# jacklishufan/InstructAny2Pix

Hardware: AMD Instinct MI355X
Metric: denoise-steps/sec (512x512, 50-step DDIM, batch 8) (higher is better)
Workload: dtype f16; 1 GPU; BASELINE configs[2]: 512x512, latent [8,4,64,64], 50-step DDIM, ctx 81 (77 text + 4 IP tokens), SDXL-base UNet + IP-Adapter; global_batch=8, parallelism=dp1, context_kv=projected in every step (reference schedule, as rounds 1-4), ranks=1, dist_backend=none (single process), weight_broadcast_route=none

## Files before the change

include/ia2p_debug.h:

```cpp
#ifndef IA2P_DEBUG_H
#define IA2P_DEBUG_H

#include "ia2p.h"

#ifdef __cplusplus
extern "C" {
#endif

void ia2p_debug_set_gemm_splitk(int splitk);
void ia2p_debug_invalidate_splitk_counters(void);
int ia2p_debug_fill_splitk_counters(void* stream, int value);
void ia2p_debug_set_splitk_inkernel(long long bytes);
void ia2p_debug_set_gn_plan(int mode);
void ia2p_debug_set_gemm_tile(int variant);
void ia2p_debug_set_xattn_min_tiles(int tiles);
void ia2p_debug_set_attn_fold(int mode);
int ia2p_debug_gemm_tile_info(int variant, int* out);
void ia2p_debug_gemm_plan(int M, int N, int K, int conv, int geglu, int* variant, int* splitk);

ia2p_status ia2p_profile_enable(ia2p_ctx* ctx, int on);
int ia2p_profile_classes(void);
ia2p_status ia2p_profile_read_prefetch(ia2p_ctx* ctx, int k, double* bytes);
ia2p_status ia2p_profile_read(ia2p_ctx* ctx, int k, char* name, int name_len, int64_t* launches, double* ms, double* flops, double* bytes);
ia2p_status ia2p_profile_read_region(ia2p_ctx* ctx, int region, int64_t* launches, double* ms, double* flops, double* bytes);
int ia2p_profile_roles(void);
ia2p_status ia2p_profile_read_role(ia2p_ctx* ctx, int role, char* name, int name_len, int64_t* launches, double* ms, double* flops, double* bytes);
ia2p_status ia2p_profile_read_role_class(ia2p_ctx* ctx, int role, int k, int64_t* launches, double* ms);

#ifdef __cplusplus
}
#endif
#endif
```

instructany2pix_amd/_ffi.py:

```python
from __future__ import annotations

import contextlib
import ctypes as C
import functools
import os

_HERE = os.path.dirname(os.path.abspath(__file__))
LIB_PATH = os.path.join(_HERE, "libia2p_hip.so")

IA2P_OK = 0
_STATUS_NAMES = {1: "INVALID", 2: "SHAPE", 3: "KEY", 4: "STATE", 5: "NOMEM", 6: "HIP", 7: "ARCH"}
MAX_BLOCKS = 4


class UNetConfigC(C.Structure):
    _fields_ = [
        ("in_channels", C.c_int), ("out_channels", C.c_int), ("n_blocks", C.c_int),
        ("block_out_channels", C.c_int * MAX_BLOCKS), ("transformer_layers_per_block", C.c_int * MAX_BLOCKS),
        ("num_heads", C.c_int * MAX_BLOCKS), ("layers_per_block", C.c_int), ("cross_attention_dim", C.c_int),
        ("norm_num_groups", C.c_int), ("norm_eps", C.c_float), ("addition_time_embed_dim", C.c_int),
        ("projection_class_embeddings_input_dim", C.c_int), ("time_embed_dim", C.c_int), ("time_proj_dim", C.c_int),
        ("mid_transformer_layers", C.c_int), ("num_time_ids", C.c_int),
    ]

# ... 77 lines not shown
    "ia2p_layernorm": (_I, [_P, _P, _P, _P, _P, _I, _I, _F]),
    "ia2p_gemm": (_I, [_P, _P, _P, _P, _P, _P, _I, _I, _I, _I]),
    "ia2p_gemm_splitk": (_I, [_P, _P, _P, _P, _P, _P, _I, _I, _I, _I, _P]),
    "ia2p_ffn": (_I, [_P, _P, _P, _P, _P, _P, _P, _P, _P, _I, _I, _I, _P]),
    "ia2p_fold_layernorm": (_I, [_P, _P, _P, _P, _P, _P, _P, _P, _I, _I]),
    "ia2p_gemm_ex": (_I, [_P, _P, _P, _P, _P, _P, _I, _I, _I, _I, _P, _P, _P, _I, _P]),
    "ia2p_debug_set_gemm_splitk": (None, [_I]),
    "ia2p_conv3x3": (_I, [_P, _P, _P, _P, _P, _P, _P, _I, _I, _I, _I, _I, _I, _I]),
    "ia2p_conv3x3_splitk": (_I, [_P, _P, _P, _P, _P, _P, _P, _I, _I, _I, _I, _I, _I, _P]),
    "ia2p_pack_conv3x3": (_I, [_P, _P, _P, _I, _I]),
    "ia2p_pack_conv_out": (_I, [_P, _P, _P, _I, _I]),
    "ia2p_conv3x3_cat": (_I, [_P, _P, _P, _P, _P, _P, _I, _I, _I, _I, _I, _I]),
    "ia2p_pack_geglu": (_I, [_P, _P, _P, _I, _I]),
    "ia2p_conv_in": (_I, [_P, _P, _P, _P, _P, _P, _I, _I, _I, _I, _I]),
    "ia2p_conv_out": (_I, [_P, _P, _P, _P, _P, _I, _I, _I, _I, _I]),
    "ia2p_attention": (_I, [_P, _P, _I, _P, _I, _I, _I, _I, _I, _P, _P, _I, _I, _F, _P, _P, _I, _I, _F]),
    "ia2p_qkv_self_attention": (_I, [_P, _P, _P, _P, _P, _P, _I, _I, _I, _I]),
    "ia2p_qkv_self_attention_ctx": (_I, [_P, _P, _P, _P, _P, _P, _I, _I, _I, _I, _P, _I, _I, _I, _P, _P, _P, _P, _I, _I, _P]),
    "ia2p_qproj_attention": (_I, [_P, _P, _P, _P, _P, _P, _I, _I, _I, _I, _I, _I, _P, _P, _I, _I, _F, _P, _P, _I, _I, _F]),
    "ia2p_linear_small": (_I, [_P, _P, _P, _P, _P, _I, _I, _I, _I, _I]),
    "ia2p_ip_attn_map": (_I, [_P, _P, _I, _P, _I, _P, _I, _I, _I, _I]),
    "ia2p_debug_set_gemm_tile": (None, [_I]),
    "ia2p_debug_gemm_tile_info": (_I, [_I, _P]),
    "ia2p_debug_set_xattn_min_tiles": (None, [_I]),
    "ia2p_debug_set_attn_fold": (None, [_I]),
    "ia2p_debug_set_splitk_inkernel": (None, [C.c_longlong]),
    "ia2p_debug_invalidate_splitk_counters": (None, []),
    "ia2p_debug_fill_splitk_counters": (_I, [_P, _I]),
    "ia2p_debug_gemm_plan": (None, [_I, _I, _I, _I, _I, _P, _P]),
    "ia2p_clip_create": (_I, [C.POINTER(CLIPConfigC), C.POINTER(_P)]),
    "ia2p_clip_destroy": (None, [_P]),
    "ia2p_clip_last_error": (C.c_char_p, [_P]),
    "ia2p_clip_arena_bytes": (_SZ, [_P]),
    "ia2p_clip_bind_arena": (_I, [_P, _P, _SZ]),
    "ia2p_clip_load_tensor": (_I, [_P, C.c_char_p, _P, C.POINTER(C.c_int64), _I, _P]),
    "ia2p_clip_finalize_weights": (_I, [_P]),
    "ia2p_clip_workspace_bytes": (_SZ, [_P, _I, _I]),
    "ia2p_clip_encode": (_I, [_P, _P, _P, _I, _I, _P, _P, _P, _P, _SZ]),
    "ia2p_clip_encode_embeds": (_I, [_P, _P, _P, _I, _I, _P, _P, _P, _SZ]),
    "ia2p_vit_create": (_I, [C.POINTER(ViTConfigC), C.POINTER(_P)]),
    "ia2p_vit_destroy": (None, [_P]),
    "ia2p_vit_last_error": (C.c_char_p, [_P]),
    "ia2p_vit_arena_bytes": (_SZ, [_P]),
    "ia2p_vit_tokens": (_I, [_P]),
    "ia2p_vit_bind_arena": (_I, [_P, _P, _SZ]),
    "ia2p_vit_load_tensor": (_I, [_P, C.c_char_p, _P, C.POINTER(C.c_int64), _I, _P]),
# ... 319 lines not shown
```

instructany2pix_amd/csrc/conv_halo_kernel.h:

```cpp
#pragma once
#include "gemm_epilogue.h"

template <int BN> struct HaloWaves { static constexpr int WGM = BN == 80 ? 8 : 4, WGN = BN == 80 ? 1 : 2; };

template <int BN, int GN> struct HaloSmem {
  using BS = BStage<BN, 64, 8, 1>;
  static constexpr int H_BASE = 3 * BS::BNL * 128, H_BYTES = 48 * 1024;
  static constexpr int GN_GSTAT = H_BASE + 2 * H_BYTES, GN_TBL = GN_GSTAT + 512, GN_ZERO = GN_TBL + 512, LOOP = GN ? GN_ZERO + 512 : H_BASE + 2 * H_BYTES;
  static constexpr int EPI = EpiCfg<256, BN, 3, HaloWaves<BN>::WGM, 64, HaloWaves<BN>::WGN, 1>::SMEM;
  static constexpr int SMEM = LOOP > EPI ? LOOP : EPI;
  static_assert(SMEM <= 160 * 1024, "halo-staged tile exceeds the CU's LDS");
};

struct GnOp { int step, e; };
constexpr int GN_NOPS = 32;
constexpr GnOp GN_OPS[GN_NOPS] = {{0, 0}, {0, 1}, {0, 2}, {1, 0}, {0, 3}, {1, 1}, {2, 0}, {0, 4}, {1, 2}, {2, 1}, {3, 0}, {0, 5}, {1, 3}, {2, 2}, {3, 1}, {0, 6},
                                  {1, 4}, {2, 3}, {3, 2}, {0, 7}, {1, 5}, {2, 4}, {3, 3}, {1, 6}, {2, 5}, {3, 4}, {1, 7}, {2, 6}, {3, 5}, {2, 7}, {3, 6}, {3, 7}};

template <int BN, int GN>
__device__ __forceinline__ void conv_halo_tile_body(const half_t* hA, const half_t* hW, int hM, int hN, int hK, int hlda, int hldw, int hsplitk, int hgroup_w, int hmfast, int gHo, int gWo, int gHs, int gWs,
                                                    int gUp, int gCin, int gCin2, const GemmArgs& p) {
  constexpr int BM = 256, BK = 64, NSTAGE = 3, PP = 1, WGM = HaloWaves<BN>::WGM, WGN = HaloWaves<BN>::WGN;
  constexpr int NWAVE = WGM * WGN;
  static_assert(NWAVE == 8, "ping-pong schedule: 8 waves (two groups of 4 by tile rows)");
// ... 413 lines not shown
  tile_epilogue<BM, BN, NSTAGE, WGM, BK, PP, WGN, 0, 1>(acc, tc, p, nullptr, kvr);
}

template <int BN, int GN = 0>
__global__ __launch_bounds__(512, 2) void conv_halo_f16_kernel(const half_t* hA, const half_t* hW, int hM, int hN, int hK, int hlda, int hldw, int hsk_gw, int hHoWo, int hHsWs, int hUpCin,
                                                                 int hCin2, const GemmArgs p) {
  conv_halo_tile_body<BN, GN>(hA, hW, hM, hN, hK, hlda, hldw, IA2P_SKGW_LO8(hsk_gw), IA2P_SKGW_GW(hsk_gw), IA2P_SKGW_FLAGS(hsk_gw) & 1, hHoWo & 0xffff, (int)((unsigned)hHoWo >> 16), hHsWs & 0xffff,
                              (int)((unsigned)hHsWs >> 16), hUpCin & 3, (int)((unsigned)hUpCin >> 2), hCin2, p);
}

template <int BN, int GN>
static hipError_t launch_halo_gn(const GemmArgs& a, hipStream_t s) {
  constexpr int smem = HaloSmem<BN, GN>::SMEM;
  static bool attr_set[64] = {false};
  int dev = 0;
  (void)hipGetDevice(&dev);
  if (dev < 0 || dev >= 64 || !attr_set[dev]) {
    hipError_t e = hipFuncSetAttribute((const void*)conv_halo_f16_kernel<BN, GN>, hipFuncAttributeMaxDynamicSharedMemorySize, smem);
    if (e != hipSuccess) return e;
    if (dev >= 0 && dev < 64) attr_set[dev] = true;
  }
  const int tiles = (a.M / 256) * ((a.N + BN - 1) / BN);
  GemmArgs b = a;
  ia2p_gemm_prepare(b, smem, 256, BN, true);
  if (b.gn_out && !b.vec8) return hipErrorInvalidValue;
  if (b.sk_counters && tiles > ia2p_sk_counter_capacity()) return hipErrorInvalidValue;
  if ((long)tiles * (a.splitk > 1 ? a.splitk : 1) >= (1L << 21)) return hipErrorInvalidValue;
  int sk_gw, howo, hsws;
  if (!ia2p_pack_skgw(b.splitk, b.group_w, b.m_fastest, false, &sk_gw) || !ia2p_pack_rowmap(b.Ho, b.Wo, &howo) || !ia2p_pack_rowmap(b.Hs, b.Ws, &hsws) || b.up < 0 || b.up > 3 || b.Cin < 0 || b.Cin >= (1 << 29))
    return hipErrorInvalidValue;
  hipLaunchKernelGGL((conv_halo_f16_kernel<BN, GN>), dim3(tiles * (a.splitk > 1 ? a.splitk : 1)), dim3(512), smem, s,
                     b.A, b.W, b.M, b.N, b.K, b.lda, b.ldw, sk_gw, howo, hsws, (int)((unsigned)b.up | ((unsigned)b.Cin << 2)), b.Cin2, b);
  return hipGetLastError();
}
template <int BN>
static hipError_t launch_halo(const GemmArgs& a, hipStream_t s) {
  if (!ia2p_conv_halo_ok(a) || !ia2p_conv_gn_ok(a)) return hipErrorInvalidValue;
  return a.gn.st0 ? launch_halo_gn<BN, 1>(a, s) : launch_halo_gn<BN, 0>(a, s);
}
```

instructany2pix_amd/csrc/gemm.hip:

```cpp
#include "gemm_kernel.h"
#include "conv_halo_kernel.h"
#include "gemm_geglu_kernel.h"

#include <algorithm>
#include <atomic>
#include <cmath>
#include <cstdio>
#include <cstdlib>
#include <cstring>
#include <map>
#include <mutex>
#include <string>
#include <tuple>
#include <vector>


static std::mutex g_plan_mu;
static unsigned long long g_plan_gen = 0;
static void plan_gen_bump() { std::lock_guard<std::mutex> lk(g_plan_mu); ++g_plan_gen; }
static int g_force_variant = -1;
extern "C" void ia2p_debug_set_gemm_tile(int v) { if (v != g_force_variant) plan_gen_bump(); g_force_variant = v; }
extern "C" int ia2p_debug_gemm_tile_info(int v, int* out) {
  if (v < 0 || v >= IA2P_GEMM_NVARIANT || !out) return -1;
  out[0] = IA2P_GEMM_TILES[v].bm; out[1] = IA2P_GEMM_TILES[v].bn; out[2] = IA2P_GEMM_TILES[v].stages; out[3] = IA2P_GEMM_TILES[v].halo ? 3 : IA2P_GEMM_TILES[v].pp;
// ... 62 lines not shown
#pragma unroll
        for (int r = 0; r < 4; ++r) { const float f = (float)o[r]; st1 += f; st2 += f * f; }
      }
    }
    if (hstats_out) {
#pragma unroll
      for (int o = 32; o > 0; o >>= 1) { st1 += __shfl_xor(st1, o); st2 += __shfl_xor(st2, o); }
      if (lane == 0) ((float2*)hstats_out)[m] = make_float2(st1, st2);
    }
  }
}

static long long g_sk_limit = -1;
extern "C" void ia2p_debug_set_splitk_inkernel(long long bytes) { g_sk_limit = bytes; }
bool ia2p_splitk_inkernel(int M, int N, int splitk) {
  static const size_t env_limit = getenv("IA2P_SPLITK_INKERNEL") ? (size_t)atoll(getenv("IA2P_SPLITK_INKERNEL")) : ((size_t)1 << 46);
  const size_t limit = g_sk_limit >= 0 ? (size_t)g_sk_limit : env_limit;
  return splitk > 1 && (size_t)splitk * M * N * sizeof(float) <= limit;
}
static int g_force_gn = -1;
extern "C" void ia2p_debug_set_gn_plan(int v) { if (v != g_force_gn) plan_gen_bump(); g_force_gn = v; }
static int g_force_splitk = -1;
extern "C" void ia2p_debug_set_gemm_splitk(int s) { if (s != g_force_splitk) plan_gen_bump(); g_force_splitk = s; }

static constexpr int POOL_INTS = 1 << 18, POOL_SK = POOL_INTS - 4096;
int ia2p_sk_counter_capacity() { return POOL_SK; }
static std::atomic<unsigned> g_sk_epoch{1};
void ia2p_sk_counters_invalidate() { g_sk_epoch.fetch_add(1, std::memory_order_relaxed); }
extern "C" void ia2p_debug_invalidate_splitk_counters(void) { ia2p_sk_counters_invalidate(); }
static int* pool_buffer(hipStream_t s) {
  struct Entry { int* p; unsigned epoch; };
  static std::mutex mu;
  static std::map<std::pair<int, hipStream_t>, Entry> pool;
  int dev = 0;
  if (hipGetDevice(&dev) != hipSuccess) return nullptr;
  const unsigned epoch = g_sk_epoch.load(std::memory_order_relaxed);
  const size_t bytes = (size_t)POOL_INTS * sizeof(int);
  std::lock_guard<std::mutex> lk(mu);
  auto it = pool.find({dev, s});
  if (it != pool.end()) {
    if (it->second.p && it->second.epoch != epoch) {
      if (hipMemsetAsync(it->second.p, 0, bytes, s) != hipSuccess) { (void)hipGetLastError(); return nullptr; }
      it->second.epoch = epoch;
    }
    return it->second.p;
  }
// ... 306 lines not shown
```

instructany2pix_amd/csrc/gemm_geglu_kernel.h:

```cpp
#pragma once
#include "gemm_tile.h"

struct Geglu320 {
  static constexpr int BM = 256, BN = 320, BK = 64, NWAVE = 8, WGN = 2, WM = 64, WN = 160, MR = 4, NR = 10;
  static constexpr int ROWB = 128, RPP = 8, A_PW = 4, B_PW = 5;
  static constexpr int STAGE = (BM + BN) * ROWB, RING = 2 * STAGE;
  static constexpr int HN = BN / 2, P16 = HN * 2 + 16, T16_BYTES = BM * P16;
  static constexpr int CONST_BYTES = 2 * BN * 4, LUT_BYTES = (IA2P_PHI_LUT_N * 8 + 15) & ~15, LNROW_BYTES = 2 * BM * 4;
  static_assert(T16_BYTES <= RING, "the output tile lives inside the ring");
  static constexpr int SMEM = RING + LNROW_BYTES + CONST_BYTES + LUT_BYTES;
  static_assert(SMEM <= 160 * 1024 && A_PW * NWAVE * RPP == BM && B_PW * NWAVE * RPP == BN, "LDS budget / staging split");
};

__global__ __launch_bounds__(512, 2) void gemm_geglu_f16_kernel(const half_t* hA, const half_t* hW, const float* h_ln_stats, const float* h_ln_cs, int hM, int hN, int hK, int hlda, int hldw,
                                                               int h_slots_gw, const GemmArgs p) {
  const int h_ln_slots = IA2P_SKGW_LO8(h_slots_gw), hgroup_w = IA2P_SKGW_GW(h_slots_gw), h_m_fastest = IA2P_SKGW_FLAGS(h_slots_gw) & 1;
  using G = Geglu320;
  constexpr int BM = G::BM, BN = G::BN, MR = G::MR, NR = G::NR, ROWB = G::ROWB, RPP = G::RPP, A_PW = G::A_PW, B_PW = G::B_PW, STAGE = G::STAGE, NT = G::NWAVE * 64;
  extern __shared__ __attribute__((aligned(1024))) char smem[];
  const int tid = threadIdx.x;
  const int lane = tid & 63;
  const int wave = __builtin_amdgcn_readfirstlane(tid >> 6);
  const __amdgpu_buffer_rsrc_t rs_a = __builtin_amdgcn_make_buffer_rsrc((void*)hA, 0, 0x7ffffe00, 0x00020000);
  const __amdgpu_buffer_rsrc_t rs_w = __builtin_amdgcn_make_buffer_rsrc((void*)hW, 0, 0x7ffffe00, 0x00020000);
// ... 289 lines not shown
    if (tid == 0 && p.partial) ((unsigned long long*)p.partial)[8 * blockIdx.x + 6] = __builtin_amdgcn_s_memrealtime();
    asm volatile("s_waitcnt vmcnt(0)" ::: "memory");
    __syncthreads();
    if (tid == 0 && p.partial) ((unsigned long long*)p.partial)[8 * blockIdx.x + 5] = __builtin_amdgcn_s_memrealtime();
  )
}

static inline bool ia2p_geglu320_ok(const GemmArgs& a) {
  return a.geglu && a.splitk <= 1 && !a.act && !a.residual && !a.rowvec && !a.stats_out && !a.gn_out && !a.gn.st0 && a.K >= 64 && a.K % 64 == 0 && a.M > 0 && a.M % Geglu320::BM == 0 &&
         a.N > 0 && a.N % Geglu320::BN == 0 && !a.rpb && (a.bias || a.ln_stats);
}
static hipError_t launch_geglu320(const GemmArgs& a, hipStream_t s) {
  using G = Geglu320;
  if (!ia2p_geglu320_ok(a)) return hipErrorInvalidValue;
  static bool attr_set[64] = {false};
  int dev = 0;
  (void)hipGetDevice(&dev);
  if (dev < 0 || dev >= 64 || !attr_set[dev]) {
    hipError_t e = hipFuncSetAttribute((const void*)gemm_geglu_f16_kernel, hipFuncAttributeMaxDynamicSharedMemorySize, G::SMEM);
    if (e != hipSuccess) return e;
    if (dev >= 0 && dev < 64) attr_set[dev] = true;
  }
  GemmArgs b = a;
  ia2p_gemm_prepare(b, G::SMEM, G::BM, G::BN, false);
  if (!b.vec8) return hipErrorInvalidValue;
  if (!b.phi_lut) return hipErrorOutOfMemory;
  const size_t a_rows = a.rpb ? ((size_t)a.M / a.rpb + 1) * (size_t)std::max(a.bstride, 0) + a.roff + a.rpb : (size_t)a.M;
  if (!ia2p_fits_buffer(a_rows, a.lda) || !ia2p_fits_buffer(a.N, a.ldw)) return hipErrorInvalidValue;
  if ((a.ln_stats && ((((uintptr_t)a.ln_cs) | ((uintptr_t)a.ln_bias)) & 15)) || (!a.ln_stats && (((uintptr_t)a.bias) & 7))) return hipErrorInvalidValue;
  b.splitk = 0; b.sk_counters = nullptr;
#ifndef IA2P_CLOCK_STAMP
  b.partial = nullptr;
#endif
  const int tiles = ((a.M + G::BM - 1) / G::BM) * ((a.N + G::BN - 1) / G::BN);
  if (tiles >= (1 << 21)) return hipErrorInvalidValue;
  int slots_gw;
  if (!ia2p_pack_skgw(b.ln_stats ? b.ln_slots : 0, b.group_w, b.m_fastest, b.ln_stats != nullptr, &slots_gw)) return hipErrorInvalidValue;
  hipLaunchKernelGGL(gemm_geglu_f16_kernel, dim3(tiles), dim3(512), G::SMEM, s, b.A, b.W, b.ln_stats, b.ln_cs, b.M, b.N, b.K, b.lda, b.ldw, slots_gw, b);
  return hipGetLastError();
}
```

instructany2pix_amd/csrc/gemm_kernel.h:

```cpp
#pragma once
#include "gemm_epilogue.h"

template <int BM, int BN, int NSTAGE, bool CONV, int WGM = 2, int BK = 64, int PP = 0, int WGN = 2, int XA = 0, bool SUB = false>
__device__ __forceinline__ void gemm_tile_body(const half_t* hA, const half_t* hW, const half_t* hzero, int hM, int hN, int hK, int hlda, int hldw, int hrpb, int hbstride,
                                               int hroff, int hsplitk, int hgroup_w, int hflags, const GemmArgs& p, const AttnArgs* xa, const float* pre_ln_stats = nullptr, int pre_ln_slots = 0, int bid0 = 0) {
  static_assert(PP != 1 || (WGM * WGN == 8 && (WGM == 4 || WGM == 8) && NSTAGE == 3), "ping-pong schedule: 8 waves (two groups of 4 by tile rows), 3-stage ring");
  static_assert(PP != 3 || (WGM == 4 && NSTAGE == 2 && !CONV), "two-slot ping-pong schedule: 8 waves, 2 k-tile slots");
  static_assert(PP != 2 || (WGM == 2 && WGN == 4 && NSTAGE == 2 && BK == 64 && BM == 256 && (BN == 256 || BN == 128) && XA == 0), "8-phase schedule: 256-row tiles, 2 x 4 waves, two k-tile buffers");
  constexpr int NWAVE = WGM * WGN;
  constexpr int WM = BM / WGM, WN = BN / WGN;
  constexpr int MR = WM / 16, NR = WN / 16;
  constexpr int ROWB = 2 * BK, CPR = ROWB / 16, RPP = 1024 / ROWB;
  using BS = BStage<BN, BK, NWAVE, PP>;
  constexpr int A_PW = BM / RPP / NWAVE, B_PW = BS::HI;
  constexpr bool B_UNEVEN = BS::UNEVEN;
  constexpr int BNL = BS::BNL;
  static_assert(BM % (RPP * NWAVE) == 0 && BN % 16 == 0 && WN % 16 == 0 && WM % 16 == 0, "tile / wave layout");
  constexpr int STAGE = (BM + BNL) * ROWB;
  constexpr int KSUB = BK / 32;
  extern __shared__ __attribute__((aligned(1024))) char smem[];

  int tid_ = threadIdx.x;
  if constexpr (SUB) asm volatile("" : "+v"(tid_));
  const int tid = tid_;
// ... 570 lines not shown
  )
  tile_epilogue<BM, BN, NSTAGE, WGM, BK, PP, WGN, XA, 0>(acc, tc, p, xa, kvr);
}

template <int BM, int BN, int NSTAGE, bool CONV, int WGM = 2, int BK = 64, int PP = 0, int WGN = 2>
__global__ __launch_bounds__(WGM * WGN * 64, 2) void gemm_f16_kernel(const half_t* hA, const half_t* hW, const half_t* hzero, int hM, int hN, int hK, int hlda, int hldw, int hrowmap,
                                                                         int hbstride, int hsk_gw, const GemmArgs p) {
  gemm_tile_body<BM, BN, NSTAGE, CONV, WGM, BK, PP, WGN, 0>(hA, hW, hzero, hM, hN, hK, hlda, hldw, hrowmap & 0xffff, hbstride, (int)((unsigned)hrowmap >> 16), IA2P_SKGW_LO8(hsk_gw),
                                                            IA2P_SKGW_GW(hsk_gw), IA2P_SKGW_FLAGS(hsk_gw), p, nullptr);
}
template <int BM, int BN, int NSTAGE, bool CONV, int WGM = 2, int BK = 64, int PP = 0, int WGN = 2>
static hipError_t launch_cfg(const GemmArgs& a, hipStream_t s) {
  constexpr int smem = EpiCfg<BM, BN, NSTAGE, WGM, BK, WGN, PP>::SMEM;
  static bool attr_set[64] = {false};
  int dev = 0;
  (void)hipGetDevice(&dev);
  if (dev < 0 || dev >= 64 || !attr_set[dev]) {
    hipError_t e = hipFuncSetAttribute((const void*)gemm_f16_kernel<BM, BN, NSTAGE, CONV, WGM, BK, PP, WGN>, hipFuncAttributeMaxDynamicSharedMemorySize, smem);
    if (e != hipSuccess) return e;
    if (dev >= 0 && dev < 64) attr_set[dev] = true;
  }
  const int tiles = ((a.M + BM - 1) / BM) * ((a.N + BN - 1) / BN);
  GemmArgs b = a;
  ia2p_gemm_prepare(b, smem, BM, BN, CONV);
  if (a.geglu && !b.vec8) return hipErrorInvalidValue;
  if (a.gn.st0) return hipErrorInvalidValue;
  if (a.gn_out && (!b.vec8 || a.geglu)) return hipErrorInvalidValue;
  if (a.geglu && !b.phi_lut) return hipErrorOutOfMemory;
  if (!CONV && IA2P_LIN_BUF) {
    const size_t a_rows = a.rpb ? ((size_t)a.M / a.rpb + 1) * (size_t)std::max(a.bstride, 0) + a.roff + a.rpb : (size_t)a.M;
    if (!ia2p_fits_buffer(a_rows, a.lda) || !ia2p_fits_buffer(a.N, a.ldw)) return hipErrorInvalidValue;
  }
  if (b.sk_counters && tiles > ia2p_sk_counter_capacity()) return hipErrorInvalidValue;
  const int extra = (!PP && a.pf && a.pf_bytes >= 4096) ? a.pf_blocks : 0;
  if ((long)tiles * (a.splitk > 1 ? a.splitk : 1) + extra >= (1L << 21)) return hipErrorInvalidValue;
  int rowmap, sk_gw;
  if (!ia2p_pack_rowmap(b.rpb, b.roff, &rowmap) || !ia2p_pack_skgw(b.splitk, b.group_w, b.m_fastest, b.ln_stats != nullptr, &sk_gw)) return hipErrorInvalidValue;
  hipLaunchKernelGGL((gemm_f16_kernel<BM, BN, NSTAGE, CONV, WGM, BK, PP, WGN>), dim3(tiles * (a.splitk > 1 ? a.splitk : 1) + extra), dim3(WGM * WGN * 64), smem, s,
                     b.A, b.W, b.zero, b.M, b.N, b.K, b.lda, b.ldw, rowmap, b.bstride, sk_gw, b);
  return hipGetLastError();
}
```

instructany2pix_amd/csrc/gemm_tile.h:

```cpp
#pragma once
#include "common.h"
#include "attention_core.h"

#include <algorithm>
#include <cmath>
#include <cstdint>
#include <cstdlib>
#include <type_traits>

bool ia2p_splitk_inkernel(int M, int N, int splitk);
int ia2p_gemm_variant_ran(const GemmArgs& a, bool conv, int v);
int ia2p_sk_counter_capacity();
int* ia2p_sk_counters(hipStream_t s, int tiles);
void ia2p_sk_counters_invalidate();
const float* ia2p_phi_lut();

#ifndef IA2P_LIN_BUF
#define IA2P_LIN_BUF 1
#endif
#define BLDS16(rsrc, ldsptr, voff, soff) \
  __builtin_amdgcn_raw_ptr_buffer_load_lds(rsrc, (__attribute__((address_space(3))) void*)(ldsptr), 16, voff, soff, 0, 0)
#define GLDS16(gptr, ldsptr)                                                                         \
  __builtin_amdgcn_global_load_lds((const __attribute__((address_space(1))) void*)(gptr),            \
                                   (__attribute__((address_space(3))) void*)(ldsptr), 16, 0, 0)

// ... 47 lines not shown

#ifdef IA2P_CLOCK_STAMP
#define IA2P_STAMP(...) __VA_ARGS__
#ifndef IA2P_STAMP_AT
#define IA2P_STAMP_AT 0
#endif
__device__ __forceinline__ unsigned long long* stamp_base(const GemmArgs& p, int nsplit) {
  return p.stamp ? p.stamp : (nsplit == 1 ? (unsigned long long*)p.partial : nullptr);
}
__device__ __forceinline__ void stamp_put(const GemmArgs& p, int nsplit, int slot) {
  unsigned long long* b = stamp_base(p, nsplit);
  if (threadIdx.x == 0 && b) b[8 * blockIdx.x + slot] = __builtin_amdgcn_s_memrealtime();
}
#else
#define IA2P_STAMP(...)
#endif

__device__ __forceinline__ int udiv_small(int a, int b) {
  int q = (int)((float)a * __builtin_amdgcn_rcpf((float)b));
  const int r = a - q * b;
  q += (r >= b ? 1 : 0) - (r < 0 ? 1 : 0);
  return q;
}
__device__ __forceinline__ void tile_order(int bid, int tiles_m, int tiles_n, int group_w, int m_fastest, int& tm, int& tn) {
  {
    const int nwg = tiles_m * tiles_n;
    const int q = nwg >> 3, r = nwg & 7, x = bid & 7, i = bid >> 3;
    bid = (x < r ? x * (q + 1) : r * (q + 1) + (x - r) * q) + i;
  }
  if (group_w > 0) {
    const int per = tiles_m * group_w;
    const int panel = udiv_small(bid, per), r = bid - panel * per;
    const int w = min(group_w, tiles_n - panel * group_w);
    tm = udiv_small(r, w); tn = panel * group_w + (r - tm * w);
  } else if (m_fastest) { tn = udiv_small(bid, tiles_m); tm = bid - tn * tiles_m; }
  else                  { tm = udiv_small(bid, tiles_n); tn = bid - tm * tiles_n; }
}

struct TileCtx {
  int hM, hN, hK;
  int tm, tn, bm0, bn0, tiles_m, tiles_n;
  int split, nsplit;
  int h_m0;
  float ln_s1, ln_s2;
#ifdef IA2P_CLOCK_STAMP
  unsigned long long stamp_c0, stamp_r0, stamp_entry;
#endif
};

static inline int ia2p_tile_group_w(int tiles, int tiles_n, int smem, double a_over_w) {
  static const int group_mode = getenv("IA2P_TILE_GROUP") ? atoi(getenv("IA2P_TILE_GROUP")) : 2;
  if (!group_mode) return 0;
  const int smem_per_cu = 160 * 1024 / smem;
  const double resident = std::min<double>(tiles / 8.0, 32.0 * std::max(1, std::min(smem_per_cu, 2)));
  static const double gscale = ia2p_exp_env("IA2P_TILE_GROUP_SCALE") ? atof(ia2p_exp_env("IA2P_TILE_GROUP_SCALE")) : 1.0;
  const int w = (int)(gscale * std::sqrt(resident * a_over_w) + 0.5);
  return std::max(1, std::min(w, tiles_n));
}
static inline int ia2p_tile_group_w(int tiles, int tiles_n, int smem, int BM, int BN) { return ia2p_tile_group_w(tiles, tiles_n, smem, (double)BM / BN); }

static inline bool ia2p_pack_rowmap(int rpb, int roff, int* out) {
  if (rpb < 0 || rpb > 0xffff || roff < 0 || roff > 0xffff) return false;
  *out = (int)((unsigned)rpb | ((unsigned)roff << 16));
  return true;
}
static inline bool ia2p_pack_skgw(int lo8, int group_w, int m_fastest, bool has_ln, int* out) {
  if (lo8 < 0 || lo8 > 0xff || group_w < 0 || group_w > 0x3fffff) return false;
  *out = (int)((unsigned)lo8 | (m_fastest ? 0x100u : 0u) | (has_ln ? 0x200u : 0u) | ((unsigned)group_w << 10));
  return true;
}
#define IA2P_SKGW_LO8(w) ((w) & 0xff)
#define IA2P_SKGW_FLAGS(w) (((w) >> 8) & 3)
#define IA2P_SKGW_GW(w) ((int)((unsigned)(w) >> 10))

static inline void ia2p_gemm_prepare(GemmArgs& b, int smem, int BM, int BN, bool conv = false) {
  auto al16 = [](const void* q) { return (((uintptr_t)q) & 15) == 0; };
  b.vec8 = (b.ldc % 8 == 0 && al16(b.C) && (!b.bias || al16(b.bias)) && (!b.residual || (b.ldr % 8 == 0 && al16(b.residual))) &&
            (!b.rowvec || (b.rowvec_ld % 8 == 0 && al16(b.rowvec)))) ? 1 : 0;
  b.c_wt = ((ia2p_wt_mask() & 1) && (size_t)b.M * b.ldc * 2 < (size_t)0x7ffffff0) ? 1 : 0;
  b.phi_lut = b.geglu ? ia2p_phi_lut() : nullptr;
  const int tiles_n = (b.N + BN - 1) / BN;
  double a_over_w = (double)BM / BN;
  static const int group_mode = getenv("IA2P_TILE_GROUP") ? atoi(getenv("IA2P_TILE_GROUP")) : 2;
  if (conv && group_mode >= 2 && b.K > 0)
    a_over_w = BM * (1.5 * b.Cin + (b.A2 ? b.Cin2 : 0) + (b.A3 ? b.Cin3 : 0)) / ((double)BN * b.K);
  b.group_w = ia2p_tile_group_w(((b.M + BM - 1) / BM) * tiles_n, tiles_n, smem, a_over_w);
}
```

instructany2pix_amd/csrc/qxattn.hip:

```cpp
#include "gemm_kernel.h"
#include "launch_args.h"

#include <cstring>

#ifndef IA2P_QX_STAGES
#define IA2P_QX_STAGES 2
#endif
template <int MODE>
__global__ __launch_bounds__(256, 2) void qproj_xattn_kernel(const half_t* hA, const half_t* hW, const half_t* hzero, const float* h_ln_stats, int hM, int hN, int hK, int hlda, int hldw,
                                                             int h_slots_gw, const GemmArgs p, const AttnArgs xa) {
  gemm_tile_body<128, 64, IA2P_QX_STAGES, false, 2, 64, 0, 2, MODE + 1>(hA, hW, hzero, hM, hN, hK, hlda, hldw, 0, 0, 0, 0, IA2P_SKGW_GW(h_slots_gw), IA2P_SKGW_FLAGS(h_slots_gw), p, &xa, h_ln_stats,
                                                                        IA2P_SKGW_LO8(h_slots_gw));
}

bool ia2p_qproj_xattn_ok(const GemmArgs& a, const AttnArgs& x) {
  return x.Nq > 0 && x.Nq % 128 == 0 && a.M == x.B * x.Nq && a.N == x.heads * 64 && a.K >= 64 && a.K % 64 == 0 && a.splitk <= 1 && !a.rpb && !a.geglu && !a.residual && !a.rowvec &&
         !a.stats_out && !a.act && x.nseg >= 1 && x.nseg <= 2 && x.seg[0].nkeys > 0 && (x.nseg == 1 || x.seg[1].nkeys > 0) &&
         (!a.bias || ((((uintptr_t)a.bias) & 15) == 0 && a.N % 8 == 0)) && x.ldo % 8 == 0 && ((((uintptr_t)x.O) & 15) == 0) &&
         ia2p_fits_buffer(a.rpb ? ((size_t)a.M / a.rpb + 1) * (size_t)(a.bstride > 0 ? a.bstride : 0) + a.roff + a.rpb : (size_t)a.M, a.lda) && ia2p_fits_buffer(a.N, a.ldw) &&
         attn_kv_resident(x);
}

hipError_t ia2p_launch_qproj_xattn(const GemmArgs& a, const AttnArgs& x, hipStream_t s) {
  if (!ia2p_qproj_xattn_ok(a, x)) return hipErrorInvalidValue;
  constexpr int BM = 128, BN = 64, SMEM = EpiCfg<128, 64, IA2P_QX_STAGES, 2, 64, 2>::SMEM > 65536 ? EpiCfg<128, 64, IA2P_QX_STAGES, 2, 64, 2>::SMEM : 65536;
  static_assert(EpiCfg<BM, BN, IA2P_QX_STAGES, 2, 64, 2>::SMEM <= SMEM, "LDS budget");
  static bool attr_set[64] = {false};
  int dev = 0;
  (void)hipGetDevice(&dev);
  if (dev < 0 || dev >= 64 || !attr_set[dev]) {
    hipError_t e = hipFuncSetAttribute((const void*)qproj_xattn_kernel<0>, hipFuncAttributeMaxDynamicSharedMemorySize, SMEM);
    if (e == hipSuccess) e = hipFuncSetAttribute((const void*)qproj_xattn_kernel<1>, hipFuncAttributeMaxDynamicSharedMemorySize, SMEM);
    if (e == hipSuccess) e = hipFuncSetAttribute((const void*)qproj_xattn_kernel<2>, hipFuncAttributeMaxDynamicSharedMemorySize, SMEM);
    if (e != hipSuccess) return e;
    if (dev >= 0 && dev < 64) attr_set[dev] = true;
  }
  const int tiles_n = a.N / BN, tiles = (a.M / BM) * tiles_n;
  GemmArgs b = a;
  b.vec8 = 1; b.splitk = 0; b.sk_counters = nullptr;
#ifndef IA2P_CLOCK_STAMP
  b.partial = nullptr;
#endif
  b.group_w = ia2p_tile_group_w(tiles, tiles_n, SMEM, BM, BN);
  AttnArgs y = x;
  y.xcd_map = (((ia2p_wt_mask() & 8) && (size_t)x.B * x.Nq * x.ldo * 2 < (size_t)0x7ffffff0) ? 2 : 0) | (ia2p_attn_fold_enabled() ? 0 : 4);
  const int extra = (a.pf && a.pf_bytes >= 4096) ? a.pf_blocks : 0;
  int slots_gw;
  if (tiles + extra >= (1 << 21) || !ia2p_pack_skgw(b.ln_stats ? b.ln_slots : 0, b.group_w, b.m_fastest, b.ln_stats != nullptr, &slots_gw)) return hipErrorInvalidValue;
  const int mode = y.nseg == 1 ? 0 : (y.seg[1].nkeys <= 64 && y.seg[0].weight != 0.f) ? 1 : 2;
#define IA2P_QX_LAUNCH(MODE)                                                                                                                   \
  hipLaunchKernelGGL(qproj_xattn_kernel<MODE>, dim3(tiles + extra), dim3(256), SMEM, s, b.A, b.W, b.zero, b.ln_stats, b.M, b.N, b.K, b.lda, b.ldw, slots_gw, b, y)
  if (mode == 0) IA2P_QX_LAUNCH(0);
  else if (mode == 1) IA2P_QX_LAUNCH(1);
  else IA2P_QX_LAUNCH(2);
#undef IA2P_QX_LAUNCH
  return hipGetLastError();
}


__global__ __launch_bounds__(512, 2) void qkv_sattn_kernel(const half_t* hA, const half_t* hW, const half_t* hzero, const float* h_ln_stats, int hM, int hN, int hK, int hlda, int hldw,
                                                           int h_slots_gw, const GemmArgs p, const AttnArgs xa, const CtxKvArgs ck) {
#ifndef IA2P_SATTN_PP
#define IA2P_SATTN_PP 3
#endif
  gemm_tile_body<256, 192, 2, false, 4, 64, IA2P_SATTN_PP, 2, 4>(hA, hW, hzero, hM, hN, hK, hlda, hldw, 0, 0, 0, 0, IA2P_SKGW_GW(h_slots_gw), IA2P_SKGW_FLAGS(h_slots_gw), p, &xa, h_ln_stats, IA2P_SKGW_LO8(h_slots_gw));
}
// ... 20 lines not shown
  const int tn = (k.N + CK_BN - 1) / CK_BN;
  return ((k.B * k.Lt + CK_BM - 1) / CK_BM) * tn + (k.Li > 0 ? ((k.B * k.Li + CK_BM - 1) / CK_BM) * tn : 0);
}
bool ia2p_qkv_sattn_ctx_ok(const AttnArgs& x, const CtxKvSlice& k) {
  if (k.B < 1 || k.B != x.B || k.Lt < 1 || k.Li < 0 || k.L != k.Lt + k.Li || k.N < 8 || k.N % 8 || k.K < 64 || k.K % 64 || k.lda < k.K || k.ldc < k.N) return false;
  if (k.Lt > 0xffff || k.Li > 0xffff || (long)k.B * k.L >= (1L << 21)) return false;
  if (!ia2p_fits_buffer((size_t)k.B * k.L + k.L, k.lda) || !ia2p_fits_buffer(k.N, k.K)) return false;
  return (long)x.B * x.heads + ia2p_qkv_sattn_ctx_tiles(k) <= ia2p_cu_count();
}

hipError_t ia2p_launch_qkv_sattn(const GemmArgs& a, const AttnArgs& x, hipStream_t s, const CtxKvSlice* ctx) {
  if (!ia2p_qkv_sattn_ok(a, x)) return hipErrorInvalidValue;
  constexpr int SMEM = EpiCfg<256, 192, 2, 4, 64, 2, 0>::SMEM;
  static_assert(SMEM >= 96 * 1024 + (2 * 256 + 2 * 192) * 4, "K / V / Q images + row and column constants");
  constexpr int CK_SMEM = EpiCfg<CK_BM, CK_BN, 3, 4, 64, 2, 1>::SMEM;
  static_assert(CK_SMEM <= SMEM, "a context K/V tile runs in the fused tile's LDS request");
  CtxKvArgs ck;
  memset(&ck, 0, sizeof ck);
  if (ctx) {
    if (!ia2p_qkv_sattn_ctx_ok(x, *ctx) || !ctx->ctx || !ctx->Wt || !ctx->Ct || (ctx->Li > 0 && (!ctx->Wi || !ctx->Ci))) return hipErrorInvalidValue;
    const int tn = (ctx->N + CK_BN - 1) / CK_BN;
    auto fill = [&](GemmArgs& g, const half_t* W, half_t* C, int rows, int roff) {
      g = gemm_desc(a.zero, ctx->ctx, ctx->lda, W, ctx->K, nullptr, nullptr, 0, C, ctx->ldc, ctx->B * rows, ctx->N, ctx->K, 0, rows, ctx->L, roff);
      ia2p_gemm_prepare(g, CK_SMEM, CK_BM, CK_BN);
    };
    fill(ck.g[0], ctx->Wt, ctx->Ct, ctx->Lt, 0);
    ck.nt[0] = ((ck.g[0].M + CK_BM - 1) / CK_BM) * tn;
    if (ctx->Li > 0) {
      fill(ck.g[1], ctx->Wi, ctx->Ci, ctx->Li, ctx->Lt);
      ck.nt[1] = ((ck.g[1].M + CK_BM - 1) / CK_BM) * tn;
    }
  }
  static bool attr_set[64] = {false};
  int dev = 0;
  (void)hipGetDevice(&dev);
  if (dev < 0 || dev >= 64 || !attr_set[dev]) {
    hipError_t e = hipFuncSetAttribute((const void*)qkv_sattn_kernel, hipFuncAttributeMaxDynamicSharedMemorySize, SMEM);
    if (e != hipSuccess) return e;
    if (dev >= 0 && dev < 64) attr_set[dev] = true;
  }
  const int tiles_n = x.heads, tiles = x.B * tiles_n;
  GemmArgs b = a;
  b.vec8 = 1; b.splitk = 0; b.sk_counters = nullptr;
#ifndef IA2P_CLOCK_STAMP
  b.partial = nullptr;
#endif
  b.m_fastest = 0;
  b.group_w = ia2p_tile_group_w(tiles, tiles_n, SMEM, 256, 192);
  AttnArgs y = x;
  y.seg[0].nkeys = 256; y.seg[0].weight = 1.f; y.nseg = 1;
  y.xcd_map = ((ia2p_wt_mask() & 8) && (size_t)x.B * x.Nq * x.ldo * 2 < (size_t)0x7ffffff0) ? 2 : 0;
  const int extra = (a.pf && a.pf_bytes >= 4096) ? a.pf_blocks : 0;
  const int nct = ck.nt[0] + ck.nt[1];
  int slots_gw;
  if (tiles + nct + extra >= (1 << 21) || !ia2p_pack_skgw(b.ln_stats ? b.ln_slots : 0, b.group_w, b.m_fastest, b.ln_stats != nullptr, &slots_gw)) return hipErrorInvalidValue;
  hipLaunchKernelGGL(qkv_sattn_kernel, dim3(tiles + nct + extra), dim3(512), SMEM, s, b.A, b.W, b.zero, b.ln_stats, b.M, b.N, b.K, b.lda, b.ldw, slots_gw, b, y, ck);
  return hipGetLastError();
}
```

Measured before the change: 55.05 steps/s.

## Choose GEMM tile-group width by exact simulation of resident panel traffic

Adds a host-side search that simulates which tile rows and columns are resident per XCD wave for each candidate group width, then picks the width that minimizes estimated A/W panel fetch bytes. This is now the default (mode 3) and replaces the closed-form sqrt rule. Residency is derived from LDS use and thread count per launch, and results are cached per shape. It also factors the tile map into a shared host/device header and adds debug probes. The risk is host-side cost on first use, and mispredicted grouping that could raise L2 traffic for some shapes.

```diff
diff --git a/include/ia2p_debug.h b/include/ia2p_debug.h
--- a/include/ia2p_debug.h
+++ b/include/ia2p_debug.h
@@ -15,6 +15,10 @@
 void ia2p_debug_set_gemm_tile(int variant);
 void ia2p_debug_set_xattn_min_tiles(int tiles);
 void ia2p_debug_set_attn_fold(int mode);
+void ia2p_debug_set_tile_group(int mode);
+void ia2p_debug_set_tile_group_w(int w);
+int ia2p_debug_tile_order(void* stream, int tiles_m, int tiles_n, int group_w, int m_fastest, int* out);
+int ia2p_debug_tile_order_host(int tiles_m, int tiles_n, int group_w, int m_fastest, int* out);
 int ia2p_debug_gemm_tile_info(int variant, int* out);
 void ia2p_debug_gemm_plan(int M, int N, int K, int conv, int geglu, int* variant, int* splitk);
 
diff --git a/instructany2pix_amd/_ffi.py b/instructany2pix_amd/_ffi.py
--- a/instructany2pix_amd/_ffi.py
+++ b/instructany2pix_amd/_ffi.py
@@ -123,6 +123,10 @@
     "ia2p_ip_attn_map": (_I, [_P, _P, _I, _P, _I, _P, _I, _I, _I, _I]),
     "ia2p_debug_set_gemm_tile": (None, [_I]),
     "ia2p_debug_gemm_tile_info": (_I, [_I, _P]),
+    "ia2p_debug_set_tile_group": (None, [_I]),
+    "ia2p_debug_set_tile_group_w": (None, [_I]),
+    "ia2p_debug_tile_order": (_I, [_P, _I, _I, _I, _I, _P]),
+    "ia2p_debug_tile_order_host": (_I, [_I, _I, _I, _I, _P]),
     "ia2p_debug_set_xattn_min_tiles": (None, [_I]),
     "ia2p_debug_set_attn_fold": (None, [_I]),
     "ia2p_debug_set_splitk_inkernel": (None, [C.c_longlong]),
diff --git a/instructany2pix_amd/csrc/conv_halo_kernel.h b/instructany2pix_amd/csrc/conv_halo_kernel.h
--- a/instructany2pix_amd/csrc/conv_halo_kernel.h
+++ b/instructany2pix_amd/csrc/conv_halo_kernel.h
@@ -459,7 +459,7 @@
   }
   const int tiles = (a.M / 256) * ((a.N + BN - 1) / BN);
   GemmArgs b = a;
-  ia2p_gemm_prepare(b, smem, 256, BN, true);
+  ia2p_gemm_prepare(b, smem, 512, 256, BN, true);
   if (b.gn_out && !b.vec8) return hipErrorInvalidValue;
   if (b.sk_counters && tiles > ia2p_sk_counter_capacity()) return hipErrorInvalidValue;
   if ((long)tiles * (a.splitk > 1 ? a.splitk : 1) >= (1L << 21)) return hipErrorInvalidValue;
diff --git a/instructany2pix_amd/csrc/gemm.hip b/instructany2pix_amd/csrc/gemm.hip
--- a/instructany2pix_amd/csrc/gemm.hip
+++ b/instructany2pix_amd/csrc/gemm.hip
@@ -108,6 +108,30 @@
 extern "C" void ia2p_debug_set_gn_plan(int v) { if (v != g_force_gn) plan_gen_bump(); g_force_gn = v; }
 static int g_force_splitk = -1;
 extern "C" void ia2p_debug_set_gemm_splitk(int s) { if (s != g_force_splitk) plan_gen_bump(); g_force_splitk = s; }
+static int g_tile_group = -1;
+extern "C" void ia2p_debug_set_tile_group(int mode) { g_tile_group = mode; }
+int ia2p_tile_group_mode() {
+  static const int env_mode = getenv("IA2P_TILE_GROUP") ? atoi(getenv("IA2P_TILE_GROUP")) : 3;
+  return g_tile_group >= 0 ? g_tile_group : env_mode;
+}
+static int g_tile_group_w = -1;
+extern "C" void ia2p_debug_set_tile_group_w(int w) { g_tile_group_w = w; }
+int ia2p_tile_group_forced_w() { return g_tile_group_w; }
+__global__ __launch_bounds__(64) void tile_order_probe_kernel(int tiles_m, int tiles_n, int group_w, int m_fastest, int* out) {
+  int tm, tn;
+  tile_order(blockIdx.x, tiles_m, tiles_n, group_w, m_fastest, tm, tn);
+  if (threadIdx.x == 0) { out[2 * blockIdx.x] = tm; out[2 * blockIdx.x + 1] = tn; }
+}
+extern "C" int ia2p_debug_tile_order(void* stream, int tiles_m, int tiles_n, int group_w, int m_fastest, int* out) {
+  if (tiles_m < 1 || tiles_n < 1 || (long)tiles_m * tiles_n >= (1L << 21) || group_w < 0 || !out) return -1;
+  hipLaunchKernelGGL(tile_order_probe_kernel, dim3(tiles_m * tiles_n), dim3(64), 0, (hipStream_t)stream, tiles_m, tiles_n, group_w, m_fastest, out);
+  return hipGetLastError() == hipSuccess ? 0 : -1;
+}
+extern "C" int ia2p_debug_tile_order_host(int tiles_m, int tiles_n, int group_w, int m_fastest, int* out) {
+  if (tiles_m < 1 || tiles_n < 1 || (long)tiles_m * tiles_n >= (1L << 21) || group_w < 0 || !out) return -1;
+  for (int b = 0; b < tiles_m * tiles_n; ++b) ia2p_tile_map_host(b, tiles_m, tiles_n, group_w, m_fastest, out[2 * b], out[2 * b + 1]);
+  return 0;
+}
 
 static constexpr int POOL_INTS = 1 << 18, POOL_SK = POOL_INTS - 4096;
 int ia2p_sk_counter_capacity() { return POOL_SK; }
diff --git a/instructany2pix_amd/csrc/gemm_geglu_kernel.h b/instructany2pix_amd/csrc/gemm_geglu_kernel.h
--- a/instructany2pix_amd/csrc/gemm_geglu_kernel.h
+++ b/instructany2pix_amd/csrc/gemm_geglu_kernel.h
@@ -335,7 +335,7 @@
     if (dev >= 0 && dev < 64) attr_set[dev] = true;
   }
   GemmArgs b = a;
-  ia2p_gemm_prepare(b, G::SMEM, G::BM, G::BN, false);
+  ia2p_gemm_prepare(b, G::SMEM, 512, G::BM, G::BN, false);
   if (!b.vec8) return hipErrorInvalidValue;
   if (!b.phi_lut) return hipErrorOutOfMemory;
   const size_t a_rows = a.rpb ? ((size_t)a.M / a.rpb + 1) * (size_t)std::max(a.bstride, 0) + a.roff + a.rpb : (size_t)a.M;
diff --git a/instructany2pix_amd/csrc/gemm_kernel.h b/instructany2pix_amd/csrc/gemm_kernel.h
--- a/instructany2pix_amd/csrc/gemm_kernel.h
+++ b/instructany2pix_amd/csrc/gemm_kernel.h
@@ -616,7 +616,7 @@
   }
   const int tiles = ((a.M + BM - 1) / BM) * ((a.N + BN - 1) / BN);
   GemmArgs b = a;
-  ia2p_gemm_prepare(b, smem, BM, BN, CONV);
+  ia2p_gemm_prepare(b, smem, WGM * WGN * 64, BM, BN, CONV);
   if (a.geglu && !b.vec8) return hipErrorInvalidValue;
   if (a.gn.st0) return hipErrorInvalidValue;
   if (a.gn_out && (!b.vec8 || a.geglu)) return hipErrorInvalidValue;
diff --git a/instructany2pix_amd/csrc/gemm_tile.h b/instructany2pix_amd/csrc/gemm_tile.h
--- a/instructany2pix_amd/csrc/gemm_tile.h
+++ b/instructany2pix_amd/csrc/gemm_tile.h
@@ -1,6 +1,8 @@
 #pragma once
 #include "common.h"
 #include "attention_core.h"
+#define IA2P_TILE_HD __host__ __device__ __forceinline__
+#include "tile_map.h"
 
 #include <algorithm>
 #include <cmath>
@@ -94,19 +96,11 @@
   q += (r >= b ? 1 : 0) - (r < 0 ? 1 : 0);
   return q;
 }
+struct TileDivSmall {
+  __device__ __forceinline__ int operator()(int a, int b) const { return udiv_small(a, b); }
+};
 __device__ __forceinline__ void tile_order(int bid, int tiles_m, int tiles_n, int group_w, int m_fastest, int& tm, int& tn) {
-  {
-    const int nwg = tiles_m * tiles_n;
-    const int q = nwg >> 3, r = nwg & 7, x = bid & 7, i = bid >> 3;
-    bid = (x < r ? x * (q + 1) : r * (q + 1) + (x - r) * q) + i;
-  }
-  if (group_w > 0) {
-    const int per = tiles_m * group_w;
-    const int panel = udiv_small(bid, per), r = bid - panel * per;
-    const int w = min(group_w, tiles_n - panel * group_w);
-    tm = udiv_small(r, w); tn = panel * group_w + (r - tm * w);
-  } else if (m_fastest) { tn = udiv_small(bid, tiles_m); tm = bid - tn * tiles_m; }
-  else                  { tm = udiv_small(bid, tiles_n); tn = bid - tm * tiles_n; }
+  ia2p_tile_map(bid, tiles_m, tiles_n, group_w, m_fastest, tm, tn, TileDivSmall());
 }
 
 struct TileCtx {
@@ -120,16 +114,15 @@
 #endif
 };
 
-static inline int ia2p_tile_group_w(int tiles, int tiles_n, int smem, double a_over_w) {
-  static const int group_mode = getenv("IA2P_TILE_GROUP") ? atoi(getenv("IA2P_TILE_GROUP")) : 2;
-  if (!group_mode) return 0;
-  const int smem_per_cu = 160 * 1024 / smem;
-  const double resident = std::min<double>(tiles / 8.0, 32.0 * std::max(1, std::min(smem_per_cu, 2)));
+int ia2p_tile_group_forced_w();
+int ia2p_tile_group_mode();
+static inline int ia2p_tile_group_w(int tiles_m, int tiles_n, int smem, int threads, double a_over_w) {
+  const int group_mode = ia2p_tile_group_mode();
+  if (group_mode && ia2p_tile_group_forced_w() > 0) return std::max(1, std::min(ia2p_tile_group_forced_w(), tiles_n));
   static const double gscale = ia2p_exp_env("IA2P_TILE_GROUP_SCALE") ? atof(ia2p_exp_env("IA2P_TILE_GROUP_SCALE")) : 1.0;
-  const int w = (int)(gscale * std::sqrt(resident * a_over_w) + 0.5);
-  return std::max(1, std::min(w, tiles_n));
+  return ia2p_tile_group_w_rule(group_mode, gscale, tiles_m, tiles_n, smem, threads, a_over_w);
 }
-static inline int ia2p_tile_group_w(int tiles, int tiles_n, int smem, int BM, int BN) { return ia2p_tile_group_w(tiles, tiles_n, smem, (double)BM / BN); }
+static inline int ia2p_tile_group_w(int tiles_m, int tiles_n, int smem, int threads, int BM, int BN) { return ia2p_tile_group_w(tiles_m, tiles_n, smem, threads, (double)BM / BN); }
 
 static inline bool ia2p_pack_rowmap(int rpb, int roff, int* out) {
   if (rpb < 0 || rpb > 0xffff || roff < 0 || roff > 0xffff) return false;
@@ -145,7 +138,7 @@
 #define IA2P_SKGW_FLAGS(w) (((w) >> 8) & 3)
 #define IA2P_SKGW_GW(w) ((int)((unsigned)(w) >> 10))
 
-static inline void ia2p_gemm_prepare(GemmArgs& b, int smem, int BM, int BN, bool conv = false) {
+static inline void ia2p_gemm_prepare(GemmArgs& b, int smem, int threads, int BM, int BN, bool conv = false) {
   auto al16 = [](const void* q) { return (((uintptr_t)q) & 15) == 0; };
   b.vec8 = (b.ldc % 8 == 0 && al16(b.C) && (!b.bias || al16(b.bias)) && (!b.residual || (b.ldr % 8 == 0 && al16(b.residual))) &&
             (!b.rowvec || (b.rowvec_ld % 8 == 0 && al16(b.rowvec)))) ? 1 : 0;
@@ -153,8 +146,7 @@
   b.phi_lut = b.geglu ? ia2p_phi_lut() : nullptr;
   const int tiles_n = (b.N + BN - 1) / BN;
   double a_over_w = (double)BM / BN;
-  static const int group_mode = getenv("IA2P_TILE_GROUP") ? atoi(getenv("IA2P_TILE_GROUP")) : 2;
-  if (conv && group_mode >= 2 && b.K > 0)
+  if (conv && ia2p_tile_group_mode() >= 2 && b.K > 0)
     a_over_w = BM * (1.5 * b.Cin + (b.A2 ? b.Cin2 : 0) + (b.A3 ? b.Cin3 : 0)) / ((double)BN * b.K);
-  b.group_w = ia2p_tile_group_w(((b.M + BM - 1) / BM) * tiles_n, tiles_n, smem, a_over_w);
+  b.group_w = ia2p_tile_group_w((b.M + BM - 1) / BM, tiles_n, smem, threads, a_over_w);
 }
diff --git a/instructany2pix_amd/csrc/qxattn.hip b/instructany2pix_amd/csrc/qxattn.hip
--- a/instructany2pix_amd/csrc/qxattn.hip
+++ b/instructany2pix_amd/csrc/qxattn.hip
@@ -41,7 +41,7 @@
 #ifndef IA2P_CLOCK_STAMP
   b.partial = nullptr;
 #endif
-  b.group_w = ia2p_tile_group_w(tiles, tiles_n, SMEM, BM, BN);
+  b.group_w = ia2p_tile_group_w(a.M / BM, tiles_n, SMEM, 256, BM, BN);
   AttnArgs y = x;
   y.xcd_map = (((ia2p_wt_mask() & 8) && (size_t)x.B * x.Nq * x.ldo * 2 < (size_t)0x7ffffff0) ? 2 : 0) | (ia2p_attn_fold_enabled() ? 0 : 4);
   const int extra = (a.pf && a.pf_bytes >= 4096) ? a.pf_blocks : 0;
@@ -108,7 +108,7 @@
     const int tn = (ctx->N + CK_BN - 1) / CK_BN;
     auto fill = [&](GemmArgs& g, const half_t* W, half_t* C, int rows, int roff) {
       g = gemm_desc(a.zero, ctx->ctx, ctx->lda, W, ctx->K, nullptr, nullptr, 0, C, ctx->ldc, ctx->B * rows, ctx->N, ctx->K, 0, rows, ctx->L, roff);
-      ia2p_gemm_prepare(g, CK_SMEM, CK_BM, CK_BN);
+      ia2p_gemm_prepare(g, CK_SMEM, 0, CK_BM, CK_BN);
     };
     fill(ck.g[0], ctx->Wt, ctx->Ct, ctx->Lt, 0);
     ck.nt[0] = ((ck.g[0].M + CK_BM - 1) / CK_BM) * tn;
@@ -132,7 +132,7 @@
   b.partial = nullptr;
 #endif
   b.m_fastest = 0;
-  b.group_w = ia2p_tile_group_w(tiles, tiles_n, SMEM, 256, 192);
+  b.group_w = ia2p_tile_group_w(x.B, tiles_n, SMEM, 512, 256, 192);
   AttnArgs y = x;
   y.seg[0].nkeys = 256; y.seg[0].weight = 1.f; y.nseg = 1;
   y.xcd_map = ((ia2p_wt_mask() & 8) && (size_t)x.B * x.Nq * x.ldo * 2 < (size_t)0x7ffffff0) ? 2 : 0;
diff --git a/instructany2pix_amd/csrc/tile_map.h b/instructany2pix_amd/csrc/tile_map.h
--- /dev/null
+++ b/instructany2pix_amd/csrc/tile_map.h
@@ -0,0 +1,105 @@
+#pragma once
+
+#include <algorithm>
+#include <cmath>
+#include <map>
+#include <mutex>
+#include <tuple>
+#include <vector>
+
+#ifndef IA2P_TILE_HD
+#define IA2P_TILE_HD inline
+#endif
+
+template <class Div>
+IA2P_TILE_HD void ia2p_tile_map(int bid, int tiles_m, int tiles_n, int group_w, int m_fastest, int& tm, int& tn, Div div) {
+  {
+    const int nwg = tiles_m * tiles_n;
+    const int q = nwg >> 3, r = nwg & 7, x = bid & 7, i = bid >> 3;
+    bid = (x < r ? x * (q + 1) : r * (q + 1) + (x - r) * q) + i;
+  }
+  if (group_w > 0) {
+    const int per = tiles_m * group_w;
+    const int panel = div(bid, per), r = bid - panel * per;
+    const int left = tiles_n - panel * group_w;
+    const int w = group_w < left ? group_w : left;
+    tm = div(r, w); tn = panel * group_w + (r - tm * w);
+  } else if (m_fastest) { tn = div(bid, tiles_m); tm = bid - tn * tiles_m; }
+  else                  { tm = div(bid, tiles_n); tn = bid - tm * tiles_n; }
+}
+
+struct Ia2pHostDiv {
+  int operator()(int a, int b) const { return a / b; }
+};
+static inline void ia2p_tile_map_host(int bid, int tiles_m, int tiles_n, int group_w, int m_fastest, int& tm, int& tn) {
+  ia2p_tile_map(bid, tiles_m, tiles_n, group_w, m_fastest, tm, tn, Ia2pHostDiv());
+}
+
+static inline void ia2p_tile_panels(int tiles_m, int tiles_n, int group_w, int m_fastest, int resident, long* rows, long* cols) {
+  std::vector<int> seen_m((size_t)tiles_m, -1), seen_n((size_t)tiles_n, -1);
+  const int tiles = tiles_m * tiles_n;
+  if (resident < 1) resident = 1;
+  long nr = 0, nc = 0;
+  int stamp = 0;
+  for (int x = 0; x < 8; ++x)
+    for (int b0 = x; b0 < tiles; b0 += 8 * resident, ++stamp)
+      for (int i = 0, b = b0; i < resident && b < tiles; ++i, b += 8) {
+        int tm, tn;
+        ia2p_tile_map_host(b, tiles_m, tiles_n, group_w, m_fastest, tm, tn);
+        if (seen_m[tm] != stamp) { seen_m[tm] = stamp; ++nr; }
+        if (seen_n[tn] != stamp) { seen_n[tn] = stamp; ++nc; }
+      }
+  *rows = nr; *cols = nc;
+}
+
+static inline int ia2p_tile_group_w_closed(int tiles, int tiles_n, int resident, double a_over_w, double scale) {
+  const double res = std::min<double>(tiles / 8.0, resident);
+  const int w = (int)(scale * std::sqrt(res * a_over_w) + 0.5);
+  return std::max(1, std::min(w, tiles_n));
+}
+
+static inline int ia2p_tile_group_w_exact(int tiles_m, int tiles_n, double row_bytes, double col_bytes, int resident, int w_closed, double* bytes_out = nullptr) {
+  typedef std::tuple<int, int, double, double, int, int> Key;
+  static std::mutex mu;
+  static std::map<Key, std::pair<int, double>> cache;
+  const Key key(tiles_m, tiles_n, row_bytes, col_bytes, resident, w_closed);
+  {
+    std::lock_guard<std::mutex> g(mu);
+    auto it = cache.find(key);
+    if (it != cache.end()) { if (bytes_out) *bytes_out = it->second.second; return it->second.first; }
+  }
+  int best = std::max(1, std::min(w_closed, tiles_n));
+  double best_bytes = -1.0;
+  if (tiles_m > 0 && tiles_n > 0 && (double)tiles_m * tiles_n * tiles_n <= (double)(1 << 26)) {
+    for (int w = 1; w <= tiles_n; ++w) {
+      long r, c;
+      ia2p_tile_panels(tiles_m, tiles_n, w, 0, resident, &r, &c);
+      const double bytes = r * row_bytes + c * col_bytes;
+      const int d = std::abs(w - w_closed), db = std::abs(best - w_closed);
+      if (best_bytes < 0 || bytes < best_bytes || (bytes == best_bytes && d < db)) { best = w; best_bytes = bytes; }
+    }
+  } else if (tiles_m > 0 && tiles_n > 0) {
+    long r, c;
+    ia2p_tile_panels(tiles_m, tiles_n, best, 0, resident, &r, &c);
+    best_bytes = r * row_bytes + c * col_bytes;
+  }
+  {
+    std::lock_guard<std::mutex> g(mu);
+    cache[key] = std::make_pair(best, best_bytes);
+  }
+  if (bytes_out) *bytes_out = best_bytes;
+  return best;
+}
+
+static inline int ia2p_tile_resident(int smem, int threads) {
+  const int by_lds = 160 * 1024 / std::max(smem, 1), by_waves = 2048 / std::max(threads, 64);
+  return 32 * std::max(1, std::min(by_lds, by_waves));
+}
+static inline int ia2p_tile_group_w_rule(int mode, double scale, int tiles_m, int tiles_n, int smem, int threads, double a_over_w) {
+  if (!mode) return 0;
+  const int smem_per_cu = 160 * 1024 / std::max(smem, 1);
+  const int resident = 32 * std::max(1, std::min(smem_per_cu, 2));
+  const int w = ia2p_tile_group_w_closed(tiles_m * tiles_n, tiles_n, resident, a_over_w, mode >= 3 ? 1.0 : scale);
+  const bool exact = mode >= 3 && threads > 0 && tiles_m > 0 && tiles_n > 0;
+  return exact ? ia2p_tile_group_w_exact(tiles_m, tiles_n, a_over_w, 1.0, ia2p_tile_resident(smem, threads), w) : w;
+}
```

Result: no change. 55.46 steps/s (median of 6 runs) (+0.7%).
